# ylab-hi/ChimeraLM

Hardware: AMD Instinct MI355X
Metric: reads/sec (whole node), 8192-bp reads batch=256 (higher is better)
Workload: dtype fp16c

## Files before the change

### chimeralm_amd/csrc/clm_api.hip

```cpp
#include <cstdio>
#include <cstdlib>
#include <cmath>
#include <cstring>
#include <map>
#include <algorithm>
#include <string>
#include <vector>

#include "chimeralm_hip.h"
#include "clm_common.h"

using namespace clm;

namespace clm {
bool debug_flag(const char* name) {
    const char* e = std::getenv("CLM_DEBUG");
    if (!e) return false;
    const size_t n = std::strlen(name);
    for (const char* p = e; *p;) {
        const char* q = std::strchr(p, ',');
        const size_t len = q ? (size_t)(q - p) : std::strlen(p);
        if (len == n && std::strncmp(p, name, n) == 0) return true;
        p += len + (q ? 1 : 0);
    }
// ... 349 lines not shown
    for (int i = 0; i < WS_N; ++i) grow |= need[i] > h->ws_cap[i];
    if (!h->edge_bnd) HIPCHK(h, hipMalloc((void**)&h->edge_bnd, (size_t)1024 * 2 * D3 * sizeof(float2)));
    if (!grow) return CLM_OK;
    HIPCHK(h, hipStreamSynchronize(st));
    for (int i = 0; i < WS_N; ++i) {
        if (need[i] <= h->ws_cap[i]) continue;
        void** p = ws_slot(h, i);
        if (*p) HIPCHK(h, hipFree(*p));
        *p = nullptr;
        h->ws_cap[i] = 0;
        HIPCHK(h, hipMalloc(p, need[i]));
        h->ws_cap[i] = need[i];
        if (i == WS_Z || i == WS_Y || i == WS_YLO) HIPCHK(h, hipMemset(*p, 0, need[i]));
    }
    return CLM_OK;
}

int ensure_filters(clm_handle* h, int L, hipStream_t st, FilterSet** out, const ReversedFilter** krev_out) {
    *krev_out = nullptr;
    const int S = conv_segments_for(L);
    const int logn = S > 1 ? 14 : conv_logn_for(L);
    if (logn < 0 || L > h->cfg.max_seq_len)
        return fail(h, CLM_E_UNSUPPORTED, "sequence length " + std::to_string(L) + " tokens exceeds max_seq_len " +
                                              std::to_string(h->cfg.max_seq_len));
    const int key = S > 1 ? KEY_LONG : logn;
    FilterSet* fs = nullptr;
    for (auto& f : h->filters)
        if (f.key == key) fs = &f;
    const int N = 1 << logn;
    if (!fs) {
        HIPCHK(h, hipStreamSynchronize(st));
        FilterSet f;
        f.key = key;
        f.logn = logn;
        f.Lf = S > 1 ? h->cfg.max_seq_len : std::min(N / 2 + 1, h->cfg.max_seq_len);
        f.KS = S > 1 ? conv_segments_for(h->cfg.max_seq_len) : 1;
        double2* scratch = nullptr;
        HIPCHK(h, hipMalloc((void**)&scratch, (size_t)D * N * sizeof(double2)));
        HIPCHK(h, hipMalloc((void**)&f.tw, (size_t)(N / 2) * sizeof(float2)));
        launch_twiddles(f.tw, logn, st);
        for (int i = 0; i < NLAYER; ++i) {
            HIPCHK(h, hipMalloc((void**)&f.ktime[i], (size_t)f.Lf * D * 4));
            HIPCHK(h, hipMalloc((void**)&f.kf[i], (size_t)D * f.KS * N * sizeof(float2)));
            std::string p = "bb.layers." + std::to_string(i) + ".mixer.filter_fn.";
            launch_filter(W(h, p + "pos_emb.z"), W(h, p + "pos_emb.t"), W(h, p + "implicit_filter.0.weight"),
                          W(h, p + "implicit_filter.0.bias"), W(h, p + "implicit_filter.1.freq"),
                          W(h, p + "implicit_filter.2.weight"), W(h, p + "implicit_filter.2.bias"),
                          W(h, p + "implicit_filter.4.weight"), W(h, p + "implicit_filter.4.bias"),
                          W(h, p + "implicit_filter.6.weight"), W(h, p + "modulation.deltas"), f.ktime[i], f.Lf, st);
            if (S == 1) {
                launch_filter_spectrum(f.ktime[i], W(h, p + "bias"), f.kf[i], scratch, f.Lf, logn, 0, f.Lf, -1, st);
                if (logn == 14) {
                    HIPCHK(h, hipMalloc((void**)&f.kfp[i], (size_t)D * N * sizeof(float2)));
                    launch_spectrum_lanepack(f.kf[i], f.kfp[i], 1, 0, st);
                }
            } else {
                float2* tmp = nullptr;
                HIPCHK(h, hipMalloc((void**)&tmp, (size_t)D * N * sizeof(float2)));
                for (int j = 0; j < f.KS; ++j) {
                    launch_filter_spectrum(f.ktime[i], W(h, p + "bias"), tmp, scratch, f.Lf, logn, j * SEG_LEN, SEG_LEN,
                                           (j - 1) * SEG_LEN, st);
                    launch_spectrum_lanepack(tmp, f.kf[i], f.KS, j, st);
                }
                HIPCHK(h, hipStreamSynchronize(st));
                HIPCHK(h, hipFree(tmp));
            }
        }
        HIPCHK(h, hipGetLastError());
        HIPCHK(h, hipStreamSynchronize(st));
        HIPCHK(h, hipFree(scratch));
        h->filters.push_back(f);
        fs = &h->filters.back();
    }
    if (conv_lone_tail(L)) {
        for (auto& r : fs->krev)
            if (r.L == L) *krev_out = &r;
        if (!*krev_out) {
            ReversedFilter r;
            r.L = L;
            r.stride = round_up(L, 8);
            for (int i = 0; i < NLAYER; ++i) {
                std::string p = "bb.layers." + std::to_string(i) + ".mixer.filter_fn.";
                HIPCHK(h, hipMalloc((void**)&r.p[i], (size_t)D * r.stride * 4));
                launch_filter_reversed(fs->ktime[i], W(h, p + "bias"), r.p[i], L, r.stride, st);
            }
            fs->krev.push_back(r);
            *krev_out = &fs->krev.back();
        }
    }
    *out = fs;
    return CLM_OK;
}

struct StageTimer {
    clm_handle* h;
    hipStream_t st;
    int stage;
    bool on;
    hipEvent_t e0{}, e1{};
    StageTimer(clm_handle* h_, hipStream_t st_, int stage_) : h(h_), st(st_), stage(stage_), on(h_->prof) {
        if (!on) return;
        if (h->recs.size() > 200000) { on = false; return; }
        if (!h->free_events.empty()) {
            e0 = h->free_events.back().first;
            e1 = h->free_events.back().second;
            h->free_events.pop_back();
        } else if (hipEventCreate(&e0) != hipSuccess || hipEventCreate(&e1) != hipSuccess) {
// ... 881 lines not shown
```

### chimeralm_amd/csrc/clm_common.h

```cpp
#pragma once
#include <hip/hip_runtime.h>
#include <stdint.h>

#include <atomic>
#include <cstdio>
#include <type_traits>

namespace clm {

constexpr int D = 256;
constexpr int D3 = 768;
constexpr int DI = 1024;
constexpr int XCDS = 8;
constexpr int NLAYER = 4;
constexpr int VOCAB = 16;
constexpr int FORDER = 64;
constexpr int EMB = 5;
constexpr int HH = 512;
constexpr int NCLS = 2;

using f32x16 = float __attribute__((ext_vector_type(16)));
using bf16x8 = __bf16 __attribute__((ext_vector_type(8)));
using f16x8 = _Float16 __attribute__((ext_vector_type(8)));
using u16x8 = unsigned short __attribute__((ext_vector_type(8)));
// ... 210 lines not shown
void launch_prefix_fill_h(const int* p0, float* h, const float* t_h, int B, int L, int Lmain, hipStream_t st);
__host__ __device__ inline int tail_range_len(int total, int grid) { return (total + grid - 1) / grid; }
int tail16_grid(int total_tiles);
void launch_gated_patch(int prec, const TailArgs& m, hipStream_t st);
void launch_fir_table(const float* short_w , const float* short_b, const float* in_bias, float4* fir , hipStream_t st);
constexpr int NEXT_NONE = 0, NEXT_INPROJ = 1, NEXT_SCORE = 2;
struct LoneTokenArgs {
    const void* y;
    float* h;
    const unsigned char* ids8;
    const float* emb;
    const float *w_out, *b_out, *ln2_g, *ln2_b, *w_fc1, *b_fc1, *w_fc2, *b_fc2;
    int last;
    const float *n_g, *n_b, *n_w, *n_bias;
    const float4* n_fir;
    const float2* edge_read;
    void* n_z;
    const float *att_w1, *att_b1, *att_w2, *att_b2;
    float *scores, *partial;
    float* ws;
    int B, L, Lp, ntiles;
    float eps;
    const unsigned char* ylo;
    int zlo;
};
size_t lone_token_ws_floats(int B);
void launch_lone_token(int prec, const LoneTokenArgs& a, hipStream_t st);
void launch_tail16(int prec, const TailArgs& m, int next, hipStream_t st);
void tail16_dump_stamps();
void conv_dump_stamps();
size_t packed_weight_bytes(int prec, int n, int k);
void launch_pack_weight(int prec, const float* w, void* out, int n, int k, hipStream_t st);

constexpr int SEG_LEN = 8192;
int conv_logn_for(int L);
int conv_segments_for(int L);
bool conv_lone_tail(int L);
void launch_filter_reversed(const float* k , const float* dskip, float* krev, int L, int stride, hipStream_t st);
void launch_filter(const float* z , const float* t , const float* w0, const float* b0,
                   const float* freq, const float* w2, const float* b2, const float* w4, const float* b4,
                   const float* w6, const float* deltas, float* k_out , int L, hipStream_t st);
void launch_filter_spectrum(const float* k , const float* dskip , float2* kf,
                            double2* scratch, int L, int logn, int seg_off, int seg_len, int prev_off, hipStream_t st);
void launch_twiddles(float2* tw, int logn, hipStream_t st);
constexpr int CONV_ONESHOT = 1;
constexpr int CONV_NO_XCD = 2;
constexpr int CONV_GATED = 4;
void launch_hyena_conv(int prec, const void* z, void* y, const float2* kf, const float2* tw, const float* ktime,
                       const float* short_w, const float* short_b, int B, int L, int Lp, int logn,
                       const unsigned char* ids8, const float* ztab, hipStream_t st, int flags = 0,
                       const float2* kf_packed = nullptr ,
                       unsigned char* ylo = nullptr );
void launch_spectrum_lanepack(const float2* src, float2* dst, int KS, int j, hipStream_t st);
void launch_ztab(const float* emb, const float* g, const float* bta, const float* w, const float* bias, float* ztab,
                 float eps, hipStream_t st);

constexpr int SEG_DOT_THREADS = 512;
struct SegPrefix {
    const int* p0 = nullptr;
    const float2* tab = nullptr;
    int tab_segs = 0;
    const int* perm = nullptr;
    const float* dots_in = nullptr;
    float* dots_out = nullptr;
    int dots_segs = 0;
};
void launch_hyena_conv_seg(int prec, const void* z, void* y, const float2* kf, int KS ,
                           const float2* tw, const float* short_w,
                           const float* short_b, float2* gscratch, int B, int L, int Lp, int S,
                           const float* krev , int krev_stride,
                           const unsigned char* ids8 , const float* ztab,
                           hipStream_t st, int flags = 0, unsigned char* ylo = nullptr ,
                           const SegPrefix& pfx = SegPrefix{});
void launch_spectra_pair_form(float2* table, int S_T, hipStream_t st);

void launch_softmax_stats(const float* scores, float* stats , int B, int L, hipStream_t st);
constexpr int POOL_SPLIT = 16;
void launch_pool(const float* h, const float* g, const float* b, const float* scores, const float* stats,
                 float* partial , int B, int L, float eps, hipStream_t st);
struct HeadW {
    const float *w0t, *b0, *w3t, *b3, *w60t, *b60, *w63t, *b63, *wot, *bo;
};
void launch_head_mlp(const float* partial, const HeadW& hw, float* pooled_out, float* logits, int B, hipStream_t st);
constexpr int POOL_PSTRIDE = 264;
void launch_score_pool16(int prec, const float* h, const float* g, const float* bta, const void* w1, const float* b1,
                         const float* w2, const float* b2, float* scores, float* partial ,
                         int B, int L, float eps, hipStream_t st);
void launch_head_tiles(const float* partial, int ntiles, const HeadW& hw, float* pooled_out, float* logits, int B,
                       hipStream_t st);
void launch_transpose(const float* in, float* out, int rows, int cols, hipStream_t st);

}
```

### chimeralm_amd/csrc/fft_core.h

```cpp
#pragma once

#if defined(__HIPCC__)
#include <hip/hip_runtime.h>
#define CLM_HD __host__ __device__ __forceinline__
#define CLM_HDC __host__ __device__ constexpr
namespace clmfft {
using V2 = float __attribute__((ext_vector_type(2)));
CLM_HD V2 make_v2(float a, float b) { return V2{a, b}; }
CLM_HD V2 splat2(float a) { return V2{a, a}; }
}
#else
#include <cmath>
#define CLM_HD inline
#define CLM_HDC constexpr
struct float2 {
    float x, y;
};
static inline float2 make_float2(float x, float y) { return float2{x, y}; }
namespace clmfft {
struct V2 {
    float x, y;
};
inline V2 operator+(V2 a, V2 b) { return V2{a.x + b.x, a.y + b.y}; }
inline V2 operator-(V2 a, V2 b) { return V2{a.x - b.x, a.y - b.y}; }
// ... 135 lines not shown
        for (int p = 0; p < 16; ++p) t[p] = v[p];
#pragma unroll
        for (int k1 = 0; k1 < 4; ++k1)
#pragma unroll
            for (int k2 = 0; k2 < 4; ++k2) v[4 * k1 + k2] = t[k1 + 4 * k2];
    }
};

template <bool INV>
struct Dft16Lo {
    template <class C>
    static CLM_HD void run(C* v) {
#pragma unroll
        for (int n1 = 0; n1 < 4; ++n1) dft4_lo<INV>(v[n1], v[n1 + 4], v[n1 + 8], v[n1 + 12]);
#pragma unroll
        for (int n1 = 1; n1 < 4; ++n1)
#pragma unroll
            for (int k2 = 1; k2 < 4; ++k2) v[n1 + 4 * k2] = mul_w16<INV>(v[n1 + 4 * k2], n1 * k2);
#pragma unroll
        for (int k2 = 0; k2 < 4; ++k2) dft4<INV>(v[4 * k2], v[4 * k2 + 1], v[4 * k2 + 2], v[4 * k2 + 3]);
        C t[16];
#pragma unroll
        for (int p = 0; p < 16; ++p) t[p] = v[p];
#pragma unroll
        for (int k1 = 0; k1 < 4; ++k1)
#pragma unroll
            for (int k2 = 0; k2 < 4; ++k2) v[4 * k1 + k2] = t[k1 + 4 * k2];
    }
};

template <bool INV>
struct Dft16HalfOut {
    template <class C>
    static CLM_HD void run(C* v) {
#pragma unroll
        for (int n1 = 0; n1 < 4; ++n1) dft4<INV>(v[n1], v[n1 + 4], v[n1 + 8], v[n1 + 12]);
#pragma unroll
        for (int n1 = 1; n1 < 4; ++n1)
#pragma unroll
            for (int k2 = 1; k2 < 4; ++k2) v[n1 + 4 * k2] = mul_w16<INV>(v[n1 + 4 * k2], n1 * k2);
        C x[9];
#pragma unroll
        for (int k2 = 0; k2 < 4; ++k2) {
            const C a0 = v[4 * k2], a1 = v[4 * k2 + 1], a2 = v[4 * k2 + 2], a3 = v[4 * k2 + 3];
            const C t0 = C::add(a0, a2), t1 = C::sub(a0, a2), t2 = C::add(a1, a3), t3 = C::template mul_mi<INV>(C::sub(a1, a3));
            x[k2] = C::add(t0, t2);
            x[4 + k2] = C::add(t1, t3);
            if (k2 == 0) x[8] = C::sub(t0, t2);
        }
#pragma unroll
        for (int q = 0; q < 9; ++q) v[q] = x[q];
    }
};

template <int R, class C>
CLM_HD void apply_twiddle_powers(C* v, C w1) {
    if (R >= 2) v[1] = C::mul(v[1], w1);
    if (R >= 4) {
        C w2 = C::mul(w1, w1), w3 = C::mul(w2, w1);
        v[2] = C::mul(v[2], w2);
        v[3] = C::mul(v[3], w3);
        if (R >= 8) {
            C w4 = C::mul(w2, w2), w5 = C::mul(w4, w1), w6 = C::mul(w4, w2), w7 = C::mul(w4, w3);
            v[4] = C::mul(v[4], w4);
            v[5] = C::mul(v[5], w5);
            v[6] = C::mul(v[6], w6);
            v[7] = C::mul(v[7], w7);
            if (R >= 16) {
                C w8 = C::mul(w4, w4);
                v[8] = C::mul(v[8], w8);
                v[9] = C::mul(v[9], C::mul(w8, w1));
                v[10] = C::mul(v[10], C::mul(w8, w2));
                v[11] = C::mul(v[11], C::mul(w8, w3));
                v[12] = C::mul(v[12], C::mul(w8, w4));
                v[13] = C::mul(v[13], C::mul(w8, w5));
                v[14] = C::mul(v[14], C::mul(w8, w6));
                v[15] = C::mul(v[15], C::mul(w8, w7));
            }
        }
    }
}

template <int LOGN>
struct Plan {
    static constexpr int N = 1 << LOGN;
    static constexpr int NPASS = (LOGN + 3) / 4;
    static constexpr int LAST = (LOGN % 4 == 0) ? 16 : (1 << (LOGN % 4));
    static constexpr int NT = (N / 32 < 64) ? 64 : N / 32;
    static constexpr int radix(int pass) { return pass < NPASS - 1 ? 16 : LAST; }
};

template <int LOGN, int R, bool INV>
CLM_HD float2 twiddle_for(int jb, int Ns, const float2* tw) {
    constexpr int N = 1 << LOGN;
    if (Ns <= 1) return make_float2(1.f, 0.f);
    float2 w1 = tw[(jb & (Ns - 1)) * (N / (Ns * R))];
    return INV ? cconj(w1) : w1;
}

template <int R, bool INV, class C>
CLM_HD void butterfly_w(C* v, bool has_tw, C w1) {
    if (has_tw) apply_twiddle_powers<R>(v, w1);
    Dft<R, INV>::run(v);
}

template <int LOGN, int R>
// ... 11 lines not shown
```

### chimeralm_amd/csrc/fft_passes.h

```cpp
#pragma once
#include "fft_core.h"

namespace clmfft {

template <int LOGN, int R>
struct PassGeom {
    static constexpr int N = 1 << LOGN;
    static constexpr int NB = N / R;
    static constexpr int NT = Plan<LOGN>::NT;
    static constexpr int IT = (NB + NT - 1) / NT;
    static constexpr int NP = (IT + 1) / 2;
    static_assert(NP * R <= 16, "a thread holds at most 16 complex pairs");
    static CLM_HD int jba(int tid, int p) { return tid + (2 * p) * NT; }
    static CLM_HD int jbb(int tid, int p) { return tid + (2 * p + 1) * NT; }
    static constexpr bool FULL = (NB % NT == 0);
    static CLM_HD bool has_a(int tid, int p) { return FULL || jba(tid, p) < NB; }
    static CLM_HD bool has_b(int tid, int p) { return 2 * p + 1 < IT && (FULL || jbb(tid, p) < NB); }
    static_assert(NT % 32 == 0, "lane distance is a whole number of padding periods");
    static CLM_HDC int pb_of(int pa) { return pa + pad_offset(NT); }
};

template <int LOGN, int R>
CLM_HD void pass_load(const float* re, const float* im, Cx2* v, int tid) {
    using G = PassGeom<LOGN, R>;
// ... 83 lines not shown
    const float2 one = make_float2(1.f, 0.f);
#pragma unroll
    for (int p = 0; p < G::NP; ++p)
        w[p] = pack2(G::has_a(tid, p) ? twiddle_for<LOGN, R, INV>(G::jba(tid, p), Ns, tw) : one,
                     G::has_b(tid, p) ? twiddle_for<LOGN, R, INV>(G::jbb(tid, p), Ns, tw) : one);
}

template <int LOGN, int R, bool INV>
CLM_HD void pass_compute_w(Cx2* v, int tid, bool has_tw, const Cx2* w) {
    using G = PassGeom<LOGN, R>;
#pragma unroll
    for (int p = 0; p < G::NP; ++p) butterfly_w<R, INV>(v + p * R, has_tw, w[p]);
}

template <int LOGN, int R>
CLM_HD void spectrum_fetch(Cx2* kv, int tid, const float2* kf) {
    using G = PassGeom<LOGN, R>;
    const float2 zero = make_float2(0.f, 0.f);
#pragma unroll
    for (int p = 0; p < G::NP; ++p) {
        const bool ha = G::has_a(tid, p), hb = G::has_b(tid, p);
#pragma unroll
        for (int q = 0; q < R; ++q)
            kv[p * R + q] = pack2(ha ? kf[stockham_in<LOGN, R>(G::jba(tid, p), q)] : zero,
                                  hb ? kf[stockham_in<LOGN, R>(G::jbb(tid, p), q)] : zero);
    }
}

template <int LOGN, int R>
CLM_HD void spectrum_multiply_and_first_inverse_v(Cx2* v, int tid, const Cx2* kv, float tail_re = 0.f, float tail_im = 0.f) {
    using G = PassGeom<LOGN, R>;
    static_assert(((1 << LOGN) / R) % 2 == 0 && G::NT % 2 == 0, "bin parity == thread parity");
    const float sg = (tid & 1) ? -1.f : 1.f;
    const Cx2 tl{splat2(sg * tail_re), splat2(sg * tail_im)};
#pragma unroll
    for (int p = 0; p < G::NP; ++p) {
#pragma unroll
        for (int q = 0; q < R; ++q) v[p * R + q] = Cx2::mul(Cx2::add(v[p * R + q], tl), kv[p * R + q]);
        Dft<R, true>::run(v + p * R);
    }
}

template <int LOGN>
struct TwLayout {
    using P = Plan<LOGN>;
    static constexpr int NP16 = PassGeom<LOGN, 16>::NP;
    static constexpr int NPL = PassGeom<LOGN, P::LAST>::NP;
    static constexpr int fwd(int p) { return (p - 1) * NP16; }
    static constexpr int fwd_last() { return (P::NPASS - 2) * NP16; }
    static constexpr int inv(int p) { return (P::NPASS - 2) * NP16 + NPL + (p - 1) * NP16; }
    static constexpr int TOTAL = (2 * P::NPASS - 3) * NP16 + NPL;
};

}
```

### chimeralm_amd/csrc/hyena_conv.hip

```cpp
#include <cstdio>
#include <cstdlib>
#include <type_traits>
#include <vector>

#include "clm_common.h"
#include "fft_passes.h"

namespace clm {
using namespace clmfft;

__global__ __launch_bounds__(64) void filter_kernel(const float* __restrict__ z, const float* __restrict__ tn,
                                                    const float* __restrict__ w0, const float* __restrict__ b0,
                                                    const float* __restrict__ freq, const float* __restrict__ w2,
                                                    const float* __restrict__ b2, const float* __restrict__ w4,
                                                    const float* __restrict__ b4, const float* __restrict__ w6,
                                                    const float* __restrict__ deltas, float* __restrict__ k_out,
                                                    int L) {
    __shared__ double hbuf[2][FORDER];
    const int t = blockIdx.x, j = threadIdx.x;
    const double f = (double)freq[j];
    double acc = (double)b0[j];
#pragma unroll
    for (int e = 0; e < EMB; ++e) acc += (double)w0[j * EMB + e] * (double)z[(size_t)t * EMB + e];
    hbuf[0][j] = sin(f * acc);
// ... 596 lines not shown
    }

    T* yA = y + ((size_t)bA * D + c) * Lp;
    T* yB = y + ((size_t)(hasB ? bB : bA) * D + c) * Lp;
    unsigned char* ylA = LO ? ylo + ((size_t)bA * D + c) * Lp : nullptr;
    unsigned char* ylB = LO ? ylo + ((size_t)(hasB ? bB : bA) * D + c) * Lp : nullptr;
#pragma unroll
    for (int ch = 0; ch < CH; ++ch) {
        const int t0 = 8 * (tid + ch * NT);
        if (t0 < HALF && t0 < Lp) {
            float oA[8], oB[8];
            lds_load8(bre + pad_index(t0), oA);
            lds_load8(bim + pad_index(t0), oB);
            if (tail && t0 == 0) {
                const float kl = ktime[(size_t)(L - 1) * D + c];
                oA[0] -= kl * gtail[0];
                oB[0] -= kl * gtail[1];
            }
#pragma unroll
            for (int e = 0; e < 8; ++e) {
                const bool ok = t0 + e < L;
                oA[e] = ok ? oA[e] * x0A[ch][e] : 0.f;
                oB[e] = ok ? oB[e] * x0B[ch][e] : 0.f;
            }
            ystore8<T, LO>(yA + t0, ylA + t0, oA);
            if (hasB) ystore8<T, LO>(yB + t0, ylB + t0, oB);
        }
    }
    if (tail && tid == TAIL_TID) {
        ystore1<T, LO>(yA + HALF, ylA + HALF, bre[pad_index(HALF)] * x0At);
        if (hasB) ystore1<T, LO>(yB + HALF, ylB + HALF, bim[pad_index(HALF)] * x0Bt);
    }
    CLM_STAMP_AT(11);
    if (STAMP && threadIdx.x == 0)
        stamps[((size_t)blockIdx.y * gridDim.x + blockIdx.x) * CONV_NSTAMP + 6] = __builtin_amdgcn_s_memrealtime();
#undef CLM_STAMP_AT
}


template <typename T, bool IDS, bool GATED = false, bool LO = false>
struct ConvGateRaw {
    Raw<T> r[GATED ? 1 : 2][2][GATED ? 1 : 2];
    T ztail[2][2];
    uint2 idd[2][2];
    unsigned short idp[2][2];
    unsigned char idt[2];
    uint4 g[2][2];
    T gtail[2];
    uint2 gl[2][2];
    unsigned char gltail[2];
};

template <typename T, bool IDS, bool GATED = false, bool LO = false>
__global__ __launch_bounds__(Plan<14>::NT) void hyena_conv_pers_kernel(
    const T* __restrict__ z, T* __restrict__ y, const float2* __restrict__ kf , const float2* __restrict__ tw,
    const float* __restrict__ ktime, const float* __restrict__ short_w, const float* __restrict__ short_b, int B, int L,
    int Lp, const unsigned char* __restrict__ ids8, const float* __restrict__ ztab, int use_xcd, unsigned char* __restrict__ ylo) {
    static_assert(!LO || std::is_same<T, f16_t>::value, "lo bytes exist in the compensated fp16 mode only");
    constexpr int LOGN = 14;
    using P = Plan<LOGN>;
    using TL = TwLayout<LOGN>;
    constexpr int N = P::N, NT = P::NT, LAST = P::LAST, HALF = N / 2, CH = 2;
    static_assert(HALF / 8 / NT == CH, "two 8-token chunks per thread");
    constexpr int TAIL_TID = HALF / 8 - 1 - (CH - 1) * NT;
    extern __shared__ __attribute__((aligned(16))) unsigned char smem[];
    float* bre = reinterpret_cast<float*>(smem);
    float* bim = bre + padded_size(N);
    float* gtail = bim + padded_size(N);
    float* zt = gtail + 4;

    const int tid = threadIdx.x;
    const int pairs = (B + 1) / 2, n_units = pairs * D;
    const bool tail = (L == HALF + 1);
    const bool xcd_order = use_xcd && (gridDim.x % XCDS) == 0;
    const int xcd = blockIdx.x % XCDS, wg_in_xcd = blockIdx.x / XCDS, wgs_per_xcd = gridDim.x / XCDS;
    const int first = xcd_order ? wg_in_xcd : (int)blockIdx.x, stride = xcd_order ? wgs_per_xcd : (int)gridDim.x;
    const int n_mine = xcd_order ? n_units / XCDS : n_units;
    auto unit_of = [&](int q, int& c, int& pair) {
        c = xcd_order ? XCDS * (q / pairs) + xcd : q / pairs;
        pair = q % pairs;
    };

    Cx2 wall[TL::TOTAL];
    {
        int ns = 16;
#pragma unroll
        for (int p = 1; p <= P::NPASS - 2; ++p) {
            pass_twiddles<LOGN, 16, false>(wall + TL::fwd(p), tid, ns, tw);
            ns *= 16;
        }
        pass_twiddles<LOGN, LAST, false>(wall + TL::fwd_last(), tid, ns, tw);
        ns = LAST;
#pragma unroll
        for (int p = 1; p <= P::NPASS - 1; ++p) {
            pass_twiddles<LOGN, 16, true>(wall + TL::inv(p), tid, ns, tw);
            ns *= 16;
        }
    }
    static_assert(!(GATED && IDS), "block 0 looks its rows up by token id: nothing to hand over");
    auto request_gate = [&](int q, ConvGateRaw<T, IDS, GATED, LO>& g, int ltid) {
        int c, pair;
        unit_of(q, c, pair);
        const int bA = 2 * pair, bB = (2 * pair + 1 < B) ? 2 * pair + 1 : bA;
        if constexpr (GATED) {
#pragma unroll
            for (int rd = 0; rd < 2; ++rd) {
                const T* row = z + ((size_t)(rd == 0 ? bA : bB) * D3 + D + c) * Lp;
                const unsigned char* rowl = zlo_row(z + (size_t)(rd == 0 ? bA : bB) * D3 * Lp, 1, c, Lp);
#pragma unroll
                for (int ch = 0; ch < CH; ++ch) {
                    const int t0 = 8 * (ltid + ch * NT);
                    g.g[ch][rd] = *reinterpret_cast<const uint4*>(row + (t0 < L ? t0 : 0));
                    if constexpr (LO) g.gl[ch][rd] = *reinterpret_cast<const uint2*>(rowl + (t0 < L ? t0 : 0));
                }
                g.gtail[rd] = row[(tail && ltid == TAIL_TID) ? HALF : 0];
                if constexpr (LO) g.gltail[rd] = rowl[(tail && ltid == TAIL_TID) ? HALF : 0];
            }
        } else if constexpr (IDS) {
#pragma unroll
            for (int rd = 0; rd < 2; ++rd) {
                const unsigned char* ir = ids8 + (size_t)(rd == 0 ? bA : bB) * Lp;
#pragma unroll
                for (int ch = 0; ch < CH; ++ch) {
                    const int t0 = 8 * (ltid + ch * NT);
                    const bool valid = t0 < L;
                    g.idd[ch][rd] = *reinterpret_cast<const uint2*>(ir + (valid ? t0 : 0));
                    g.idp[ch][rd] = *reinterpret_cast<const unsigned short*>(ir + ((valid && t0 > 0) ? t0 - 2 : 0));
                }
                g.idt[rd] = ir[(tail && ltid == TAIL_TID) ? HALF : 0];
            }
        } else {
#pragma unroll
            for (int rd = 0; rd < 2; ++rd) {
                const T* zr = z + (size_t)(rd == 0 ? bA : bB) * D3 * Lp;
#pragma unroll
                for (int a3 = 1; a3 < 3; ++a3) {
                    const T* row = zr + (size_t)(a3 * D + c) * Lp;
#pragma unroll
                    for (int ch = 0; ch < CH; ++ch) {
                        const int t0 = 8 * (ltid + ch * NT);
                        raw_load(g.r[ch][rd][a3 - 1], row, t0, t0 < L);
                    }
                    g.ztail[rd][a3 - 1] = row[(tail && ltid == TAIL_TID) ? HALF : 0];
                }
            }
        }
    };

    ConvGateRaw<T, IDS, GATED, LO> cur;
    request_gate(first < n_mine ? first : 0, cur, tid);

#pragma unroll 1
    for (int u = first; u < n_mine; u += stride) {
        int ltid = tid;
        asm volatile("" : "+v"(ltid));
#pragma unroll
        for (int i = 0; i < TL::TOTAL; ++i)
            asm volatile("" : "+v"(wall[i].re.x), "+v"(wall[i].re.y), "+v"(wall[i].im.x), "+v"(wall[i].im.y));
        int c, pair;
        unit_of(u, c, pair);
        const int bA = 2 * pair, bB = 2 * pair + 1;
        const bool hasB = bB < B;
        const float4* kfc = reinterpret_cast<const float4*>(kf) + (size_t)c * (N / 2);
        float sw[3][3], sb[3];
#pragma unroll
        for (int q = 0; q < 3; ++q) {
#pragma unroll
            for (int e = 0; e < 3; ++e) sw[q][e] = short_w[(q * D + c) * 3 + e];
            sb[q] = short_b[q * D + c];
        }
        if constexpr (IDS) {
            if (ltid < 48) zt[ltid] = ztab[(size_t)(ltid & 15) * D3 + (ltid >> 4) * D + c];
            __syncthreads();
        }
        const bool full_unit = L >= HALF && hasB;
        auto phase_a = [&](auto fullc) {
            constexpr bool FULL = decltype(fullc)::value;
            float gAt = 0.f, gBt = 0.f;
            if constexpr (GATED) {
#pragma unroll
                for (int ch = 0; ch < CH; ++ch) {
                    const int t0 = 8 * (ltid + ch * NT);
                    float gA[8], gB[8];
                    cvt8<T>(cur.g[ch][0], gA);
                    cvt8<T>(cur.g[ch][1], gB);
                    if constexpr (LO) {
                        add_lo8(cur.gl[ch][0], gA);
                        add_lo8(cur.gl[ch][1], gB);
                    }
                    if constexpr (!FULL) {
#pragma unroll
                        for (int e = 0; e < 8; ++e) {
                            gA[e] = t0 + e < L ? gA[e] : 0.f;
                            gB[e] = (hasB && t0 + e < L) ? gB[e] : 0.f;
                        }
                    }
                    lds_store8(bre + pad_index(t0), gA);
                    lds_store8(bim + pad_index(t0), gB);
                }
                if (tail && ltid == TAIL_TID) {
                    float l0 = 0.f, l1 = 0.f;
                    if constexpr (LO) l0 = lo1b(cur.gltail[0]), l1 = lo1b(cur.gltail[1]);
                    gtail[0] = to_float(cur.gtail[0]) + l0;
                    gtail[1] = hasB ? to_float(cur.gtail[1]) + l1 : 0.f;
                }
            } else {
#pragma unroll
            for (int ch = 0; ch < CH; ++ch) {
                const int t0 = 8 * (ltid + ch * NT);
                const bool valid = FULL ? true : t0 < L, validB = FULL ? true : (valid && hasB);
                float xa[3][10], xb[3][10], gA[8], gB[8], x1[8], v[8], x1b[8], vb[8];
                if constexpr (IDS) {
                    ids_decode<true, 6>(cur.idd[ch][0], cur.idp[ch][0], t0, valid, zt, xa);
                    ids_decode<true, 6>(cur.idd[ch][1], cur.idp[ch][1], t0, validB, zt, xb);
                } else {
#pragma unroll
                    for (int a3 = 1; a3 < 3; ++a3) {
                        raw_decode(cur.r[ch][0][a3 - 1], t0, valid, xa[a3]);
                        raw_decode(cur.r[ch][1][a3 - 1], t0, validB, xb[a3]);
                    }
                }
                fir3_pair(xa[1], xb[1], sw[1][0], sw[1][1], sw[1][2], sb[1], x1, x1b);
                fir3_pair(xa[2], xb[2], sw[2][0], sw[2][1], sw[2][2], sb[2], v, vb);
#pragma unroll
                for (int e = 0; e < 8; ++e) {
                    gA[e] = (FULL || t0 + e < L) ? v[e] * x1[e] : 0.f;
                    gB[e] = (FULL || (hasB && t0 + e < L)) ? vb[e] * x1b[e] : 0.f;
                }
                lds_store8(bre + pad_index(t0), gA);
                lds_store8(bim + pad_index(t0), gB);
                if (ch == CH - 1 && tail && ltid == TAIL_TID) {
                    float ta[3] = {0.f, 0.f, 0.f}, tb[3] = {0.f, 0.f, 0.f};
#pragma unroll
                    for (int a3 = 1; a3 < 3; ++a3) {
                        const float za = IDS ? zt[a3 * 16 + (cur.idt[0] & 15)] : to_float(cur.ztail[0][a3 - 1]);
                        const float zb = IDS ? zt[a3 * 16 + (cur.idt[1] & 15)] : to_float(cur.ztail[1][a3 - 1]);
                        ta[a3] = sb[a3] + sw[a3][0] * xa[a3][8] + sw[a3][1] * xa[a3][9] + sw[a3][2] * za;
                        tb[a3] = sb[a3] + sw[a3][0] * xb[a3][8] + sw[a3][1] * xb[a3][9] + sw[a3][2] * zb;
                    }
                    gAt = ta[1] * ta[2];
                    gBt = hasB ? tb[1] * tb[2] : 0.f;
                }
            }
            if (tail && ltid == TAIL_TID) {
                gtail[0] = gAt;
                gtail[1] = gBt;
            }
            }
        };
        if (full_unit) phase_a(std::true_type{});
        else phase_a(std::false_type{});
        __syncthreads();

        Cx2 v[16];
        {
            int Ns = 1;
#pragma unroll
            for (int p = 0; p < P::NPASS - 1; ++p) {
                if (p == 0) {
                    pass_first_lower<LOGN>(bre, bim, v, ltid);
                } else {
                    pass_load<LOGN, 16>(bre, bim, v, ltid);
                    pass_compute_w<LOGN, 16, false>(v, ltid, true, wall + TL::fwd(p));
                }
                __syncthreads();
                pass_store<LOGN, 16>(bre, bim, v, ltid, Ns);
                __syncthreads();
                Ns *= 16;
            }
        }
        {
            Cx2 kv[16];
#pragma unroll
            for (int e = 0; e < 16; ++e) {
                const float4 q4 = kfc[e * NT + ltid];
                kv[e] = Cx2{make_v2(q4.x, q4.y), make_v2(q4.z, q4.w)};
            }
            pass_load<LOGN, LAST>(bre, bim, v, ltid);
            pass_compute_w<LOGN, LAST, false>(v, ltid, true, wall + TL::fwd_last());
            spectrum_multiply_and_first_inverse_v<LOGN, LAST>(v, ltid, kv, tail ? gtail[0] : 0.f, tail ? gtail[1] : 0.f);
        }
        __syncthreads();
        pass_store<LOGN, LAST>(bre, bim, v, ltid, 1);
        __syncthreads();
        {
            int Ns = LAST;
#pragma unroll
            for (int p = 1; p < P::NPASS - 1; ++p) {
                pass_load<LOGN, 16>(bre, bim, v, ltid);
                pass_compute_w<LOGN, 16, true>(v, ltid, true, wall + TL::inv(p));
                __syncthreads();
                pass_store<LOGN, 16>(bre, bim, v, ltid, Ns);
                __syncthreads();
                Ns *= 16;
            }
        }
        Raw<T> x0r[CH][2];
        T x0tail[2];
        uint2 x0l[CH][2];
        unsigned char x0ltail[2] = {0, 0};
        const T* zA = z + (size_t)bA * D3 * Lp;
        const T* zB = z + (size_t)(hasB ? bB : bA) * D3 * Lp;
        if constexpr (GATED) {
#pragma unroll
            for (int rd = 0; rd < 2; ++rd) {
                const T* row = (rd == 0 ? zA : zB) + (size_t)c * Lp;
                const unsigned char* rowl = zlo_row(rd == 0 ? zA : zB, 0, c, Lp);
#pragma unroll
                for (int ch = 0; ch < CH; ++ch) {
                    const int t0 = 8 * (ltid + ch * NT);
                    x0r[ch][rd].d = *reinterpret_cast<const uint4*>(row + (t0 < L ? t0 : 0));
                    if constexpr (LO) x0l[ch][rd] = *reinterpret_cast<const uint2*>(rowl + (t0 < L ? t0 : 0));
                }
                x0tail[rd] = row[(tail && ltid == TAIL_TID) ? HALF : 0];
                if constexpr (LO) x0ltail[rd] = rowl[(tail && ltid == TAIL_TID) ? HALF : 0];
            }
        } else if constexpr (!IDS) {
#pragma unroll
            for (int rd = 0; rd < 2; ++rd) {
                const T* row = (rd == 0 ? zA : zB) + (size_t)c * Lp;
#pragma unroll
                for (int ch = 0; ch < CH; ++ch) {
                    const int t0 = 8 * (ltid + ch * NT);
                    raw_load(x0r[ch][rd], row, t0, t0 < L);
                }
                x0tail[rd] = row[(tail && ltid == TAIL_TID) ? HALF : 0];
            }
        }
        ConvGateRaw<T, IDS, GATED, LO> nxt;
        {
            const int un = u + stride;
            request_gate(un < n_mine ? un : u, nxt, ltid);
        }
        pass_load<LOGN, 16>(bre, bim, v, ltid);
        pass_compute_last_inverse_lower<LOGN>(v, ltid, wall + TL::inv(P::NPASS - 1));
        __syncthreads();
        pass_store_lower<LOGN>(bre, bim, v, ltid, tail);
        __syncthreads();

        auto phase_c = [&](auto fullc) {
            constexpr bool FULL = decltype(fullc)::value;
            T* yA = y + ((size_t)bA * D + c) * Lp;
            T* yB = y + ((size_t)(hasB ? bB : bA) * D + c) * Lp;
            unsigned char* ylA = LO ? ylo + ((size_t)bA * D + c) * Lp : nullptr;
            unsigned char* ylB = LO ? ylo + ((size_t)(hasB ? bB : bA) * D + c) * Lp : nullptr;
#pragma unroll
            for (int ch = 0; ch < CH; ++ch) {
                const int t0 = 8 * (ltid + ch * NT);
                const bool valid = FULL ? true : t0 < L, validB = FULL ? true : (valid && hasB);
                float xa[10] = {}, xb[10] = {}, x0a[8], x0b[8];
                if constexpr (GATED) {
                    cvt8<T>(x0r[ch][0].d, x0a);
                    cvt8<T>(x0r[ch][1].d, x0b);
                    if constexpr (LO) {
                        add_lo8(x0l[ch][0], x0a);
                        add_lo8(x0l[ch][1], x0b);
                    }
                } else if constexpr (IDS) {
                    float xa3[3][10], xb3[3][10];
#pragma unroll
                    for (int rd = 0; rd < 2; ++rd)
                        asm volatile("" : "+v"(cur.idd[ch][rd].x), "+v"(cur.idd[ch][rd].y), "+v"(cur.idp[ch][rd]));
                    ids_decode<true, 1>(cur.idd[ch][0], cur.idp[ch][0], t0, valid, zt, xa3);
                    ids_decode<true, 1>(cur.idd[ch][1], cur.idp[ch][1], t0, validB, zt, xb3);
#pragma unroll
                    for (int e = 0; e < 10; ++e) xa[e] = xa3[0][e], xb[e] = xb3[0][e];
                } else {
                    raw_decode(x0r[ch][0], t0, valid, xa);
                    raw_decode(x0r[ch][1], t0, validB, xb);
                }
                if constexpr (!GATED) fir3_pair(xa, xb, sw[0][0], sw[0][1], sw[0][2], sb[0], x0a, x0b);
                if (t0 < Lp) {
                    float oA[8], oB[8];
                    lds_load8(bre + pad_index(t0), oA);
                    lds_load8(bim + pad_index(t0), oB);
                    if (tail && t0 == 0) {
                        const float kl = ktime[(size_t)(L - 1) * D + c];
                        oA[0] -= kl * gtail[0];
                        oB[0] -= kl * gtail[1];
                    }
#pragma unroll
                    for (int e = 0; e < 8; ++e) {
                        const bool ok = FULL || t0 + e < L;
                        oA[e] = ok ? oA[e] * x0a[e] : 0.f;
                        oB[e] = ok ? oB[e] * x0b[e] : 0.f;
                    }
                    ystore8<T, LO>(yA + t0, ylA + t0, oA);
                    if (hasB) ystore8<T, LO>(yB + t0, ylB + t0, oB);
                }
                if (ch == CH - 1 && tail && ltid == TAIL_TID) {
                    float za = IDS ? zt[cur.idt[0] & 15] : to_float(x0tail[0]);
                    float zb = IDS ? zt[cur.idt[1] & 15] : to_float(x0tail[1]);
                    if constexpr (GATED && LO) za += lo1b(x0ltail[0]), zb += lo1b(x0ltail[1]);
                    const float x0At = GATED ? za : sb[0] + sw[0][0] * xa[8] + sw[0][1] * xa[9] + sw[0][2] * za;
                    const float x0Bt = GATED ? zb : sb[0] + sw[0][0] * xb[8] + sw[0][1] * xb[9] + sw[0][2] * zb;
                    ystore1<T, LO>(yA + HALF, ylA + HALF, bre[pad_index(HALF)] * x0At);
                    if (hasB) ystore1<T, LO>(yB + HALF, ylB + HALF, bim[pad_index(HALF)] * x0Bt);
                }
            }
        };
        if (full_unit) phase_c(std::true_type{});
        else phase_c(std::false_type{});
        cur = nxt;
        __syncthreads();
    }
}

template <typename T, bool IDS, bool GATED = false, bool LO = false>
static void launch_conv_pers_inst(const void* z, void* y, const float2* kf, const float2* tw, const float* ktime,
                                  const float* short_w, const float* short_b, int B, int L, int Lp, const unsigned char* ids8,
                                  const float* ztab, int use_xcd, hipStream_t st, unsigned char* ylo = nullptr) {
    using P = Plan<14>;
    constexpr size_t lds = (size_t)2 * padded_size(P::N) * sizeof(float) + 256;
    static const int cus = [] {
        int dev = 0, n = 256;
        if (hipGetDevice(&dev) == hipSuccess) (void)hipDeviceGetAttribute(&n, hipDeviceAttributeMultiprocessorCount, dev);
        return n > 0 ? n : 256;
    }();
    const int n_units = ((B + 1) / 2) * D;
    dim3 grid(n_units < cus ? n_units : cus), block(P::NT);
    launch_lds<hyena_conv_pers_kernel<T, IDS, GATED, LO>>(grid, block, lds, st, reinterpret_cast<const T*>(z), reinterpret_cast<T*>(y), kf,
                                                         tw, ktime, short_w, short_b, B, L, Lp, ids8, ztab, use_xcd, ylo);
}


typedef unsigned v4u32 __attribute__((vector_size(16)));
__device__ __forceinline__ __amdgpu_buffer_rsrc_t make_rsrc(const void* p, size_t bytes) {
    const unsigned long long a = reinterpret_cast<unsigned long long>(p);
    const unsigned lo = __builtin_amdgcn_readfirstlane((unsigned)a), hi = __builtin_amdgcn_readfirstlane((unsigned)(a >> 32));
    void* q = reinterpret_cast<void*>(((unsigned long long)hi << 32) | lo);
    return __builtin_amdgcn_make_buffer_rsrc(q, 0, __builtin_amdgcn_readfirstlane((int)bytes), 0x00020000);
}

__global__ __launch_bounds__(512) void spectrum_lanepack_kernel(const float2* __restrict__ src, float4* __restrict__ dst, int KS, int j) {
    constexpr int N = 16384, NT = 512, LAST = Plan<14>::LAST;
    static_assert(LAST == 4 && Plan<14>::NT == NT, "pair geometry of the 16384-point plan");
    const int c = blockIdx.x, t = threadIdx.x;
    const float2* s = src + (size_t)c * N;
    float4* d = dst + ((size_t)c * KS + j) * (N / 2);
#pragma unroll
    for (int e = 0; e < 16; ++e) {
        const int ka = 2 * (e / LAST) + (N / LAST / NT) * (e % LAST);
        const float2 a = s[t + NT * ka], b = s[t + NT * (ka + 1)];
        d[e * NT + t] = make_float4(a.x, b.x, a.y, b.y);
    }
}
void launch_spectrum_lanepack(const float2* src, float2* dst, int KS, int j, hipStream_t st) {
    hipLaunchKernelGGL(spectrum_lanepack_kernel, dim3(D), dim3(512), 0, st, src, reinterpret_cast<float4*>(dst), KS, j);
}

template <typename T, bool LONE, bool IDS, bool GATED = false, bool LO = false>
__global__ __launch_bounds__(Plan<14>::NT) void hyena_conv_seg_kernel(
    const T* __restrict__ z, T* __restrict__ y, const float2* __restrict__ kf ,
    int KS, const float2* __restrict__ tw, const float* __restrict__ short_w, const float* __restrict__ short_b,
    float2* __restrict__ gscratch , int B, int L, int Lp, int S,
    const float* __restrict__ krev , int krev_stride,
    const unsigned char* __restrict__ ids8 , const float* __restrict__ ztab , int use_xcd,
    unsigned char* __restrict__ ylo, const SegPrefix pfx) {
    static_assert(!LO || std::is_same<T, f16_t>::value, "lo bytes exist in the compensated fp16 mode only");
    constexpr int LOGN = 14;
    using P = Plan<LOGN>;
    using TL = TwLayout<LOGN>;
    constexpr int N = P::N, NT = P::NT, LAST = P::LAST, HALF = N / 2, CH = HALF / 8 / NT;
    static_assert(HALF == SEG_LEN && CH == 2, "segment = half transform");
    static_assert(NT == SEG_DOT_THREADS, "one partial dot product per thread in SegPrefix::dots");
    extern __shared__ __attribute__((aligned(16))) unsigned char smem[];
    float* bre = reinterpret_cast<float*>(smem);
    float* bim = bre + padded_size(N);

    const int tid = threadIdx.x;
    const int pairs = (B + 1) / 2, xcd = blockIdx.x % XCDS, slot = blockIdx.x / XCDS;
    const int c = use_xcd ? XCDS * (slot / pairs) + xcd : (int)blockIdx.x / pairs, pair = use_xcd ? slot % pairs : (int)blockIdx.x % pairs;
    const bool hasB = 2 * pair + 1 < B;
    const int bA = pfx.perm ? pfx.perm[2 * pair] : 2 * pair;
    const int bB = hasB ? (pfx.perm ? pfx.perm[2 * pair + 1] : 2 * pair + 1) : bA;
    const T* zA = z + (size_t)bA * D3 * Lp;
    const T* zB = z + (size_t)(hasB ? bB : bA) * D3 * Lp;
    T* yA = y + ((size_t)bA * D + c) * Lp;
    T* yB = y + ((size_t)(hasB ? bB : bA) * D + c) * Lp;
    unsigned char* ylA = LO ? ylo + ((size_t)bA * D + c) * Lp : nullptr;
    unsigned char* ylB = LO ? ylo + ((size_t)(hasB ? bB : bA) * D + c) * Lp : nullptr;
    const float2* kfc = kf + (size_t)c * KS * N;
    float2* gs = gscratch + ((size_t)pair * D + c) * S * N;
    const float* kr = LONE ? krev + (size_t)c * krev_stride : nullptr;
    float dotA = 0.f, dotB = 0.f;
    int m_start = 0;
    if (pfx.p0 != nullptr && hasB) {
        const int pa = pfx.p0[bA], pb = pfx.p0[bB], pm = pa < pb ? pa : pb;
        m_start = pm > 0 ? ((pm - 1) * 128) / SEG_LEN : 0;
        if (m_start > S - 1) m_start = S - 1;
    }
    m_start = __builtin_amdgcn_readfirstlane(m_start);
    if constexpr (LONE) {
        if (m_start > 0) dotA = dotB = pfx.dots_in[((size_t)c * pfx.dots_segs + (m_start - 1)) * NT + threadIdx.x];
    }

    float sw[3][3], sb[3];
#pragma unroll
    for (int q = 0; q < 3; ++q) {
#pragma unroll
        for (int e = 0; e < 3; ++e) sw[q][e] = short_w[(q * D + c) * 3 + e];
// ... 637 lines not shown
```

Before: 8257.

## Restructure persistent conv FFT into radix-32/16 passes with fewer LDS round-trips

```diff
diff --git a/chimeralm_amd/csrc/clm_api.hip b/chimeralm_amd/csrc/clm_api.hip
--- a/chimeralm_amd/csrc/clm_api.hip
+++ b/chimeralm_amd/csrc/clm_api.hip
@@ -425,7 +425,7 @@
                 launch_filter_spectrum(f.ktime[i], W(h, p + "bias"), f.kf[i], scratch, f.Lf, logn, 0, f.Lf, -1, st);
                 if (logn == 14) {
                     HIPCHK(h, hipMalloc((void**)&f.kfp[i], (size_t)D * N * sizeof(float2)));
-                    launch_spectrum_lanepack(f.kf[i], f.kfp[i], 1, 0, st);
+                    launch_spectrum_lanepack_pers(f.kf[i], f.kfp[i], st);
                 }
             } else {
                 float2* tmp = nullptr;
diff --git a/chimeralm_amd/csrc/clm_common.h b/chimeralm_amd/csrc/clm_common.h
--- a/chimeralm_amd/csrc/clm_common.h
+++ b/chimeralm_amd/csrc/clm_common.h
@@ -286,6 +286,7 @@
                        const float2* kf_packed = nullptr ,
                        unsigned char* ylo = nullptr );
 void launch_spectrum_lanepack(const float2* src, float2* dst, int KS, int j, hipStream_t st);
+void launch_spectrum_lanepack_pers(const float2* src, float2* dst, hipStream_t st);
 void launch_ztab(const float* emb, const float* g, const float* bta, const float* w, const float* bias, float* ztab,
                  float eps, hipStream_t st);
 
diff --git a/chimeralm_amd/csrc/fft_core.h b/chimeralm_amd/csrc/fft_core.h
--- a/chimeralm_amd/csrc/fft_core.h
+++ b/chimeralm_amd/csrc/fft_core.h
@@ -211,6 +211,67 @@
         for (int q = 0; q < 9; ++q) v[q] = x[q];
     }
 };
+
+
+template <bool INV, class C>
+CLM_HD C mul_w32(C v, int k) {
+    if (k % 2 == 0) return mul_w16<INV>(v, k / 2);
+    const float a = 0.98078528040323044913f, b = 0.83146961230254523708f, c = 0.55557023301960222474f,
+                d = 0.19509032201612826785f;
+    float cx, sy;
+    switch (k) {
+        case 1: cx = a; sy = d; break;
+        case 3: cx = b; sy = c; break;
+        case 5: cx = c; sy = b; break;
+        case 7: cx = d; sy = a; break;
+        case 9: cx = -d; sy = a; break;
+        case 11: cx = -c; sy = b; break;
+        case 13: cx = -b; sy = c; break;
+        default: cx = -a; sy = d; break;
+    }
+    return C::mulc(v, cx, INV ? sy : -sy);
+}
+
+template <bool INV>
+CLM_HD void dft32_combine(Cx2* v) {
+#pragma unroll
+    for (int k = 0; k < 16; ++k) {
+        const Cx1 e{v[k].re.x, v[k].im.x}, t = mul_w32<INV>(Cx1{v[k].re.y, v[k].im.y}, k);
+        v[k] = Cx2{make_v2(e.re + t.re, e.re - t.re), make_v2(e.im + t.im, e.im - t.im)};
+    }
+}
+
+template <bool INV>
+CLM_HD void dft32_combine_lower(Cx2* v) {
+#pragma unroll
+    for (int k = 0; k < 16; ++k) {
+        const Cx1 t = mul_w32<INV>(Cx1{v[k].re.y, v[k].im.y}, k);
+        if (k == 0) v[0].re.y = v[0].re.x - t.re, v[0].im.y = v[0].im.x - t.im;
+        v[k].re.x += t.re;
+        v[k].im.x += t.im;
+    }
+}
+
+CLM_HD void apply_twiddles32(Cx2* v, Cx2 t) {
+    const Cx2 x1{splat2(t.re.x), splat2(t.im.x)};
+    const Cx2 x2 = Cx2::mul(x1, x1), x4 = Cx2::mul(x2, x2), x8 = Cx2::mul(x4, x4);
+    Cx2 p[16];
+    p[0] = Cx2{make_v2(1.f, t.re.y), make_v2(0.f, t.im.y)};
+    p[1] = Cx2::mul(p[0], x1);
+    p[2] = Cx2::mul(p[0], x2);
+    p[3] = Cx2::mul(p[1], x2);
+#pragma unroll
+    for (int m = 4; m < 8; ++m) p[m] = Cx2::mul(p[m - 4], x4);
+#pragma unroll
+    for (int m = 8; m < 16; ++m) p[m] = Cx2::mul(p[m - 8], x8);
+    {
+        const Cx1 b = Cx1::mulc(Cx1{v[0].re.y, v[0].im.y}, t.re.y, t.im.y);
+        v[0].re.y = b.re;
+        v[0].im.y = b.im;
+    }
+#pragma unroll
+    for (int m = 1; m < 16; ++m) v[m] = Cx2::mul(v[m], p[m]);
+}
 
 template <int R, class C>
 CLM_HD void apply_twiddle_powers(C* v, C w1) {
diff --git a/chimeralm_amd/csrc/fft_passes.h b/chimeralm_amd/csrc/fft_passes.h
--- a/chimeralm_amd/csrc/fft_passes.h
+++ b/chimeralm_amd/csrc/fft_passes.h
@@ -159,4 +159,69 @@
     static constexpr int TOTAL = (2 * P::NPASS - 3) * NP16 + NPL;
 };
 
-}
+template <int LAST>
+CLM_HD int lanepack_bin(int e, int t) {
+    return t + 512 * (2 * (e / LAST) + (16384 / LAST / 512) * (e % LAST));
+}
+
+struct Plan32 {
+    static constexpr int LOGN = 14, N = 1 << LOGN, NT = 512;
+    static constexpr int TW_FWD1 = 0, TW_FWD2 = 1, TW_INV1 = 2, TW_INV2 = 3, TOTAL = 4;
+};
+static_assert(Plan32::NT == Plan<14>::NT && PassGeom<14, 16>::NP == 1 && PassGeom<14, 16>::FULL, "geometry shared with Plan<14>");
+
+template <bool INV>
+CLM_HD Cx2 twiddle32(int jb, int Ns, const float2* tw) {
+    const int i = (jb & (Ns - 1)) * (Plan32::N / (32 * Ns));
+    const float2 w = tw[i], w2 = tw[2 * i];
+    return INV ? pack2(cconj(w2), cconj(w)) : pack2(w2, w);
+}
+
+template <bool INV>
+CLM_HD void plan32_twiddles(Cx2* w, int tid, const float2* tw) {
+    w[Plan32::TW_FWD1] = twiddle32<false>(tid, 32, tw);
+    pass_twiddles<14, 16, false>(w + Plan32::TW_FWD2, tid, 1024, tw);
+    w[Plan32::TW_INV1] = twiddle32<true>(tid, 16, tw);
+    w[Plan32::TW_INV2] = twiddle32<true>(tid, 512, tw);
+}
+
+CLM_HD void plan32_first(const float* re, const float* im, Cx2* v, int tid) {
+    pass_first_lower<14>(re, im, v, tid);
+    dft32_combine<false>(v);
+}
+
+template <bool INV>
+CLM_HD void plan32_compute(Cx2* v, Cx2 w) {
+    apply_twiddles32(v, w);
+    Dft<16, INV>::run(v);
+    dft32_combine<INV>(v);
+}
+
+template <int NS>
+CLM_HD void plan32_store(float* re, float* im, const Cx2* v, int tid) {
+    const int k = tid & (NS - 1);
+    const int pa = pad_index((tid - k) * 32 + k);
+#pragma unroll
+    for (int q = 0; q < 16; ++q) {
+        const int oa = pad_offset(q * NS), ob = pad_offset((q + 16) * NS);
+        re[pa + oa] = v[q].re.x, im[pa + oa] = v[q].im.x;
+        re[pa + ob] = v[q].re.y, im[pa + ob] = v[q].im.y;
+    }
+}
+
+CLM_HD void plan32_compute_last_inverse_lower(Cx2* v, Cx2 w) {
+    apply_twiddles32(v, w);
+    Dft<16, true>::run(v);
+    dft32_combine_lower<true>(v);
+}
+CLM_HD void plan32_store_lower(float* re, float* im, const Cx2* v, int tid, bool keep_mid) {
+    const int pa = pad_index(tid);
+#pragma unroll
+    for (int q = 0; q < 16; ++q) {
+        const int off = pad_offset(q * 512);
+        re[pa + off] = v[q].re.x, im[pa + off] = v[q].im.x;
+    }
+    if (keep_mid && tid == 0) re[pad_index(Plan32::N / 2)] = v[0].re.y, im[pad_index(Plan32::N / 2)] = v[0].im.y;
+}
+
+}
diff --git a/chimeralm_amd/csrc/hyena_conv.hip b/chimeralm_amd/csrc/hyena_conv.hip
--- a/chimeralm_amd/csrc/hyena_conv.hip
+++ b/chimeralm_amd/csrc/hyena_conv.hip
@@ -672,15 +672,13 @@
 };
 
 template <typename T, bool IDS, bool GATED = false, bool LO = false>
-__global__ __launch_bounds__(Plan<14>::NT) void hyena_conv_pers_kernel(
+__global__ __launch_bounds__(Plan32::NT) void hyena_conv_pers_kernel(
     const T* __restrict__ z, T* __restrict__ y, const float2* __restrict__ kf , const float2* __restrict__ tw,
     const float* __restrict__ ktime, const float* __restrict__ short_w, const float* __restrict__ short_b, int B, int L,
     int Lp, const unsigned char* __restrict__ ids8, const float* __restrict__ ztab, int use_xcd, unsigned char* __restrict__ ylo) {
     static_assert(!LO || std::is_same<T, f16_t>::value, "lo bytes exist in the compensated fp16 mode only");
-    constexpr int LOGN = 14;
-    using P = Plan<LOGN>;
-    using TL = TwLayout<LOGN>;
-    constexpr int N = P::N, NT = P::NT, LAST = P::LAST, HALF = N / 2, CH = 2;
+    using P = Plan32;
+    constexpr int N = P::N, NT = P::NT, HALF = N / 2, CH = 2;
     static_assert(HALF / 8 / NT == CH, "two 8-token chunks per thread");
     constexpr int TAIL_TID = HALF / 8 - 1 - (CH - 1) * NT;
     extern __shared__ __attribute__((aligned(16))) unsigned char smem[];
@@ -701,22 +699,8 @@
         pair = q % pairs;
     };
 
-    Cx2 wall[TL::TOTAL];
-    {
-        int ns = 16;
-#pragma unroll
-        for (int p = 1; p <= P::NPASS - 2; ++p) {
-            pass_twiddles<LOGN, 16, false>(wall + TL::fwd(p), tid, ns, tw);
-            ns *= 16;
-        }
-        pass_twiddles<LOGN, LAST, false>(wall + TL::fwd_last(), tid, ns, tw);
-        ns = LAST;
-#pragma unroll
-        for (int p = 1; p <= P::NPASS - 1; ++p) {
-            pass_twiddles<LOGN, 16, true>(wall + TL::inv(p), tid, ns, tw);
-            ns *= 16;
-        }
-    }
+    Cx2 wall[P::TOTAL];
+    plan32_twiddles<false>(wall, tid, tw);
     static_assert(!(GATED && IDS), "block 0 looks its rows up by token id: nothing to hand over");
     auto request_gate = [&](int q, ConvGateRaw<T, IDS, GATED, LO>& g, int ltid) {
         int c, pair;
@@ -775,7 +759,7 @@
         int ltid = tid;
         asm volatile("" : "+v"(ltid));
 #pragma unroll
-        for (int i = 0; i < TL::TOTAL; ++i)
+        for (int i = 0; i < P::TOTAL; ++i)
             asm volatile("" : "+v"(wall[i].re.x), "+v"(wall[i].re.y), "+v"(wall[i].im.x), "+v"(wall[i].im.y));
         int c, pair;
         unit_of(u, c, pair);
@@ -873,22 +857,15 @@
         __syncthreads();
 
         Cx2 v[16];
-        {
-            int Ns = 1;
-#pragma unroll
-            for (int p = 0; p < P::NPASS - 1; ++p) {
-                if (p == 0) {
-                    pass_first_lower<LOGN>(bre, bim, v, ltid);
-                } else {
-                    pass_load<LOGN, 16>(bre, bim, v, ltid);
-                    pass_compute_w<LOGN, 16, false>(v, ltid, true, wall + TL::fwd(p));
-                }
-                __syncthreads();
-                pass_store<LOGN, 16>(bre, bim, v, ltid, Ns);
-                __syncthreads();
-                Ns *= 16;
-            }
-        }
+        plan32_first(bre, bim, v, ltid);
+        __syncthreads();
+        plan32_store<1>(bre, bim, v, ltid);
+        __syncthreads();
+        pass_load<14, 16>(bre, bim, v, ltid);
+        plan32_compute<false>(v, wall[P::TW_FWD1]);
+        __syncthreads();
+        plan32_store<32>(bre, bim, v, ltid);
+        __syncthreads();
         {
             Cx2 kv[16];
 #pragma unroll
@@ -896,25 +873,18 @@
                 const float4 q4 = kfc[e * NT + ltid];
                 kv[e] = Cx2{make_v2(q4.x, q4.y), make_v2(q4.z, q4.w)};
             }
-            pass_load<LOGN, LAST>(bre, bim, v, ltid);
-            pass_compute_w<LOGN, LAST, false>(v, ltid, true, wall + TL::fwd_last());
-            spectrum_multiply_and_first_inverse_v<LOGN, LAST>(v, ltid, kv, tail ? gtail[0] : 0.f, tail ? gtail[1] : 0.f);
-        }
-        __syncthreads();
-        pass_store<LOGN, LAST>(bre, bim, v, ltid, 1);
-        __syncthreads();
-        {
-            int Ns = LAST;
-#pragma unroll
-            for (int p = 1; p < P::NPASS - 1; ++p) {
-                pass_load<LOGN, 16>(bre, bim, v, ltid);
-                pass_compute_w<LOGN, 16, true>(v, ltid, true, wall + TL::inv(p));
-                __syncthreads();
-                pass_store<LOGN, 16>(bre, bim, v, ltid, Ns);
-                __syncthreads();
-                Ns *= 16;
-            }
-        }
+            pass_load<14, 16>(bre, bim, v, ltid);
+            pass_compute_w<14, 16, false>(v, ltid, true, wall + P::TW_FWD2);
+            spectrum_multiply_and_first_inverse_v<14, 16>(v, ltid, kv, tail ? gtail[0] : 0.f, tail ? gtail[1] : 0.f);
+        }
+        __syncthreads();
+        pass_store<14, 16>(bre, bim, v, ltid, 1);
+        __syncthreads();
+        pass_load<14, 16>(bre, bim, v, ltid);
+        plan32_compute<true>(v, wall[P::TW_INV1]);
+        __syncthreads();
+        plan32_store<16>(bre, bim, v, ltid);
+        __syncthreads();
         Raw<T> x0r[CH][2];
         T x0tail[2];
         uint2 x0l[CH][2];
@@ -952,10 +922,10 @@
             const int un = u + stride;
             request_gate(un < n_mine ? un : u, nxt, ltid);
         }
-        pass_load<LOGN, 16>(bre, bim, v, ltid);
-        pass_compute_last_inverse_lower<LOGN>(v, ltid, wall + TL::inv(P::NPASS - 1));
-        __syncthreads();
-        pass_store_lower<LOGN>(bre, bim, v, ltid, tail);
+        pass_load<14, 16>(bre, bim, v, ltid);
+        plan32_compute_last_inverse_lower(v, wall[P::TW_INV2]);
+        __syncthreads();
+        plan32_store_lower(bre, bim, v, ltid, tail);
         __syncthreads();
 
         auto phase_c = [&](auto fullc) {
@@ -1030,7 +1000,7 @@
 static void launch_conv_pers_inst(const void* z, void* y, const float2* kf, const float2* tw, const float* ktime,
                                   const float* short_w, const float* short_b, int B, int L, int Lp, const unsigned char* ids8,
                                   const float* ztab, int use_xcd, hipStream_t st, unsigned char* ylo = nullptr) {
-    using P = Plan<14>;
+    using P = Plan32;
     constexpr size_t lds = (size_t)2 * padded_size(P::N) * sizeof(float) + 256;
     static const int cus = [] {
         int dev = 0, n = 256;
@@ -1052,21 +1022,26 @@
     return __builtin_amdgcn_make_buffer_rsrc(q, 0, __builtin_amdgcn_readfirstlane((int)bytes), 0x00020000);
 }
 
+template <int LAST>
 __global__ __launch_bounds__(512) void spectrum_lanepack_kernel(const float2* __restrict__ src, float4* __restrict__ dst, int KS, int j) {
-    constexpr int N = 16384, NT = 512, LAST = Plan<14>::LAST;
-    static_assert(LAST == 4 && Plan<14>::NT == NT, "pair geometry of the 16384-point plan");
+    constexpr int N = 16384, NT = 512;
+    static_assert(Plan<14>::NT == NT && Plan32::NT == NT, "pair geometry of the 16384-point plans");
     const int c = blockIdx.x, t = threadIdx.x;
     const float2* s = src + (size_t)c * N;
     float4* d = dst + ((size_t)c * KS + j) * (N / 2);
 #pragma unroll
     for (int e = 0; e < 16; ++e) {
-        const int ka = 2 * (e / LAST) + (N / LAST / NT) * (e % LAST);
-        const float2 a = s[t + NT * ka], b = s[t + NT * (ka + 1)];
+        const int ka = lanepack_bin<LAST>(e, t);
+        const float2 a = s[ka], b = s[ka + NT];
         d[e * NT + t] = make_float4(a.x, b.x, a.y, b.y);
     }
 }
 void launch_spectrum_lanepack(const float2* src, float2* dst, int KS, int j, hipStream_t st) {
-    hipLaunchKernelGGL(spectrum_lanepack_kernel, dim3(D), dim3(512), 0, st, src, reinterpret_cast<float4*>(dst), KS, j);
+    static_assert(Plan<14>::LAST == 4, "the segmented kernel's last forward radix");
+    hipLaunchKernelGGL(spectrum_lanepack_kernel<4>, dim3(D), dim3(512), 0, st, src, reinterpret_cast<float4*>(dst), KS, j);
+}
+void launch_spectrum_lanepack_pers(const float2* src, float2* dst, hipStream_t st) {
+    hipLaunchKernelGGL(spectrum_lanepack_kernel<16>, dim3(D), dim3(512), 0, st, src, reinterpret_cast<float4*>(dst), 1, 0);
 }
 
 template <typename T, bool LONE, bool IDS, bool GATED = false, bool LO = false>
```

Result: no change. 8409, median of 6 (+1.8%).
